# HNUicda/CoIVO

Hardware: AMD Instinct MI355X
Metric: training frame-pairs/sec at 320x256 (higher is better)
Workload: dtype bf16

## Files before the change

### coivo_amd/_lib.py

```python
from __future__ import annotations

import ctypes as C
import os

_HERE = os.path.dirname(os.path.abspath(__file__))
LIB_PATH = os.environ.get("COLVO_LIB_PATH") or os.path.join(_HERE, "lib", "libcolvo.so")

F32, BF16 = 0, 1
ABI_VERSION = 17

_vp, _i, _f, _sz = C.c_void_p, C.c_int, C.c_float, C.c_size_t


class ConvDesc(C.Structure):
    _fields_ = [(n, C.c_int32) for n in (
        "dtype", "B", "Ho", "Wo", "Cout", "ksize", "stride", "relu",
        "C0", "up0", "C1", "up1", "Hi", "Wi")]


class AdamArena(C.Structure):
    _fields_ = [("param", C.c_void_p), ("grad", C.c_void_p), ("exp_avg", C.c_void_p), ("exp_avg_sq", C.c_void_p), ("n", C.c_size_t)]


class WgradSlabs(C.Structure):
    _fields_ = [("scratch", C.c_void_p), ("dw", C.c_void_p), ("db", C.c_void_p), ("nsplit", C.c_int32), ("Cout", C.c_int32),
                ("Ctot", C.c_int32), ("pad_", C.c_int32)]


AUG_ROW_FLOATS = 20
WGRAD_GROUP_MAX = 16
MAX_ARENAS = 4
ADAM_PLAIN_PER_WG = 2048


class Cmd(C.Structure):
    _fields_ = [("op", C.c_int32), ("stream", C.c_int32), ("desc", ConvDesc), ("p", C.c_void_p * 12),
                ("i", C.c_int32 * 12), ("f", C.c_float * 4)]


(CMD_CONV_FWD, CMD_CONV_DGRAD, CMD_CONV_WGRAD, CMD_PACK_NCHW, CMD_UNPACK_NHWC_GRAD, CMD_DEPTH_HEAD_FWD,
 CMD_DEPTH_HEAD_BWD, CMD_DEPTH_HEAD_WGRAD, CMD_POSE_HEAD_FWD, CMD_POSE_HEAD_BWD, CMD_FORK, CMD_JOIN,
 CMD_DEPTH_HEAD_BWD_PARTS, CMD_CONV_DGRAD_BOTH, CMD_WGRAD_REDUCE_GROUP, CMD_CONV_DGRAD_PLANES, CMD_CONV_BWD_FUSED,
# ... 7 lines not shown
    "colvo_warp_loss_fwd": (_i, [_vp] * 7 + [_i, _i, _i, _f, _vp, _vp, _vp]),
    "colvo_warp_loss_bwd": (_i, [_vp] * 7 + [_i, _i, _i, _f] + [_vp] * 8),
    "colvo_warp_loss_fused": (_i, [_vp] * 7 + [_i, _i, _i, _f] + [_vp] * 6),
    "colvo_warp_loss_fused_bwd": (_i, [_vp] * 5 + [_i, _i, _i] + [_vp] * 5),
    "colvo_warp_loss_fused_bwd_params": (_i, [_vp] * 4 + [_i] + [_vp] * 4),
    "colvo_warp_loss_rescale": (_i, [_vp, _i, _vp]),
    "colvo_warp_loss_rescale_to": (_i, [_vp, _i, _vp, _vp]),
    "colvo_inverse_warp": (_i, [_vp] * 4 + [_i] * 4 + [_vp] * 3),
    "colvo_geo_loss_workspace_floats": (_sz, [_i, _i, _i]),
    "colvo_geo_loss_fwd": (_i, [_vp] * 4 + [_i, _i, _i] + [_vp] * 3),
    "colvo_geo_loss_bwd": (_i, [_vp] * 4 + [_i, _i, _i] + [_vp] * 7),
    "colvo_smooth_loss_fwd": (_i, [_vp, _vp, _i, _i, _i, _vp, _vp, _vp]),
    "colvo_smooth_loss_bwd": (_i, [_vp, _vp, _i, _i, _i, _vp, _vp, _vp]),
    "colvo_avgpool2_fwd": (_i, [_vp, _i, _i, _i, _vp, _vp]),
    "colvo_avgpool2_bwd": (_i, [_vp, _i, _i, _i, _vp, _vp]),
    "colvo_adam_step_multi": (_i, [_vp, _i, _f, _f, _f, _f, _f, _i, _vp]),
    "colvo_zero_multi": (_i, [_vp, _vp, _i, _vp]),
    "colvo_adam_pack_step": (_i, [_i, _vp, _i, _i, _f, _f, _f, _f, _f, _vp, _i, _vp]),
    "colvo_adam_pack_step_scaled": (_i, [_i, _vp, _i, _i, _f, _f, _f, _f, _f, _vp, _vp, _i, _vp]),
    "colvo_full_objective_workspace_floats": (_sz, [_i, _i, _i, _i]),
    "colvo_full_objective_fwd": (_i, [_vp] * 8 + [_i] * 4 + [_f] * 3 + [_vp] * 3),
    "colvo_full_objective_bwd": (_i, [_vp] * 3 + [_i] * 4 + [_f, _f] + [_vp] * 6),
    "colvo_full_objective_terms": (_i, [_vp, _i, _i, _i, _i, C.POINTER(_vp)]),
    "colvo_conv_fwd": (_i, [C.POINTER(ConvDesc)] + [_vp] * 6),
    "colvo_conv_dgrad": (_i, [C.POINTER(ConvDesc), _i, _vp, _vp, _vp, _vp, _i, _vp]),
    "colvo_conv_dgrad_both": (_i, [_vp, _vp, _vp, _vp, _vp, _vp, _vp, _vp]),
    "colvo_conv_dgrad_planes": (_i, [C.POINTER(ConvDesc), _vp, _vp, _i, _i, _vp, _i, _vp]),
    "colvo_conv_head_fused_ok": (_i, [C.POINTER(ConvDesc)]),
    "colvo_conv_head_fused": (_i, [C.POINTER(ConvDesc), _vp, _vp, _vp, _vp, _vp, _f, _f, _vp, _vp, _vp, _vp]),
    "colvo_pack_stem_pose": (_i, [_vp, _i, _i, _i, _vp, _vp, _vp]),
    "colvo_conv_bwd_fused_ok": (_i, [C.POINTER(ConvDesc)]),
    "colvo_conv_bwd_fused": (_i, [C.POINTER(ConvDesc), _vp, _vp, _vp, _i, _vp, _vp, _vp, _vp, _vp, _vp, _vp]),
    "colvo_conv_bwd_fused_head_rows": (_i, [C.POINTER(ConvDesc)]),
    "colvo_depth_head_wgrad_reduce": (_i, [_vp, _i, _vp, _vp, _vp]),
    "colvo_depth_head_wgrad_mfma_rows": (_i, [_i, _i, _i]),
    "colvo_depth_head_wgrad_mfma": (_i, [_vp, _vp, _i, _i, _i, _vp, _vp]),
    "colvo_conv_wgrad": (_i, [C.POINTER(ConvDesc)] + [_vp] * 6),
    "colvo_conv_wgrad_clean": (_i, [_vp] * 6 + [_i, _vp]),
    "colvo_conv_wgrad_scratch_bytes": (_sz, [C.POINTER(ConvDesc)]),
    "colvo_conv_wgrad_det": (_i, [C.POINTER(ConvDesc)] + [_vp] * 6 + [_sz, _vp]),
    "colvo_conv_wgrad_splits": (_i, [C.POINTER(ConvDesc)]),
    "colvo_conv_wgrad_slabs": (_i, [C.POINTER(ConvDesc)] + [_vp] * 4 + [_sz, _vp]),
    "colvo_wgrad_reduce_group": (_i, [_vp, _i, _vp]),
    "colvo_depth_head_wgrad_scratch_bytes": (_sz, [_i, _i, _i, _i]),
    "colvo_depth_head_wgrad_det": (_i, [_i, _vp, _vp, _i, _i, _i, _i, _vp, _vp, _vp, _sz, _vp]),
    "colvo_pose_head_bwd_det": (_i, [_i, _vp, _vp, _vp, _vp, _vp, _vp, _vp, _i, _i, _i, _f, _f, _vp, _vp, _vp, _vp]),
    "colvo_relu_bwd_inplace": (_i, [_i, _vp, _vp, _sz, _vp]),
    "colvo_pack_weights": (_i, [_i, _vp, _i, _i, _i, _vp, _vp, _vp]),
    "colvo_pack_weights_multi": (_i, [_i, _vp, _vp, _i, _i, _vp, _vp, _vp]),
    "colvo_pack_nchw": (_i, [_i, C.POINTER(_vp), C.POINTER(C.c_int32), _i, _i, _i, _i, _i, _vp, _vp]),
    "colvo_unpack_nhwc_grad": (_i, [_i, _vp, _i, _i, _i, _i, _i, _i, _vp, _i, _vp]),
    "colvo_depth_head_fwd": (_i, [_i, _vp, _vp, _vp, _i, _i, _i, _i, _f, _f, _vp, _vp]),
    "colvo_depth_head_bwd": (_i, [_i, _vp, _vp, _vp, _vp, _i, _i, _i, _i, _f, _f, _vp, _vp, _vp, _vp, _vp]),
    "colvo_depth_head_wgrad": (_i, [_i, _vp, _vp, _i, _i, _i, _i, _vp, _vp, _vp]),
    "colvo_depth_head_bwd_parts": (_i, [_i] + [_vp] * 9 + [_i, _i, _i, _i, _f, _f] + [_vp] * 5),
    "colvo_pose_head_fwd": (_i, [_i, _vp, _vp, _vp, _i, _i, _i, _f, _f, _vp, _vp]),
    "colvo_pose_head_bwd": (_i, [_i, _vp, _vp, _vp, _vp, _vp, _vp, _vp, _i, _i, _i, _f, _f, _vp, _vp, _vp, _vp]),
    "colvo_adam_step": (_i, [_vp, _vp, _vp, _vp, _sz, _f, _f, _f, _f, _f, _vp, _vp]),
    "colvo_adam_step_t": (_i, [_vp, _vp, _vp, _vp, _sz, _f, _f, _f, _f, _f, _i, _vp]),
    "colvo_cast_f32_bf16": (_i, [_vp, _vp, _sz, _i, _vp]),
    "colvo_zero": (_i, [_vp, _sz, _vp]),
    "colvo_frames_u8_to_f32": (_i, [_vp, _i, _i, _i, _i, _i, _vp, _vp]),
    "colvo_frames_u8_augment": (_i, [_vp, _i, _i, _i, _i, _i, _vp, _vp, _vp]),
    "colvo_read_npy_u8_frames": (_i, [_vp, _i, _i, _i, _vp, _i]),
    "colvo_backproject": (_i, [_vp, _vp, _vp, _i, _i, _i, _vp, _vp]),
    "colvo_stitch_workspace_ints": (_sz, [_i, _i, _i, _i]),
# ... 112 lines not shown
```

### coivo_amd/csrc/bwd16.hip

```cpp
#define COLVO_ACC_CONSTRAINT "+v"
#include "conv_common.h"
#include "tuning.h"

namespace colvo {
namespace {

constexpr int TOH = 8, TOW = 16, PH = TOH + 2, PW = TOW + 2, NPIX = PH * PW;
constexpr int PIXB = 32;
constexpr int WROWB = 352;

struct Bwd16K {
    const char* dy;
    const char* x;
    const char* w_bwd;
    char* dx;
    float* dw;
    float* db;
    int B, H, W;
    int tiles_x, tiles_y, ntiles, tiles_per_wg;
    int relu_mask;
    const float* dpre;
    const float* head_w;
    float* head_partials;
};

constexpr int DH = PH + 2, DW = PW + 2;

#ifndef COLVO_BWD16_HEAD_WGS
#define COLVO_BWD16_HEAD_WGS 4
#endif
template <int MODE>
__global__ __launch_bounds__(NT, MODE == 2 ? 3 : MODE == 1 ? COLVO_BWD16_HEAD_WGS : 4) void k_bwd16(const Bwd16K a) {
    constexpr bool HEAD = MODE >= 1, headw = MODE == 2;
    __shared__ __attribute__((aligned(16))) char sG[NPIX * PIXB];
    __shared__ __attribute__((aligned(16))) char sX[NPIX * PIXB];
    __shared__ __attribute__((aligned(16))) char sW[16 * WROWB];
    __shared__ float sdb[NT];
    __shared__ __attribute__((aligned(16))) uint32_t sDs[HEAD ? DH * DW : 4];
    __shared__ __attribute__((aligned(16))) float sD[MODE == 2 ? DH * DW : 4];
    __shared__ __attribute__((aligned(16))) char sY[MODE == 2 ? NPIX * PIXB : 16];
    float hb = 0.0f;
    const int tid = threadIdx.x, lane = tid & 63, wave = __builtin_amdgcn_readfirstlane(tid >> 6);
    const int l15 = lane & 15, kg = lane >> 4;

    for (int i = tid; i < 16 * 10 * 2; i += NT) {
        const int half = i & 1, tap = (i >> 1) % 10, ci = i / 20;
        u32x4 v = u32x4{0u, 0u, 0u, 0u};
        if (tap < 9) v = ld16(a.w_bwd + ((ci * 9 + tap) * 16 + half * 8) * 2);
        st16(sW + ci * WROWB + tap * 32 + half * 16, v);
    }

    const int t_begin = blockIdx.x * a.tiles_per_wg;
    const int t_end = min(a.ntiles, t_begin + a.tiles_per_wg);
    const int tiles_per_img = a.tiles_x * a.tiles_y;
    const long long img_bytes = (long long)a.H * a.W * 16 * 2;
    const long long tot_bytes = img_bytes * a.B;
    const __amdgpu_buffer_rsrc_t rdy = __builtin_amdgcn_make_buffer_rsrc((void*)a.dy, 0, (int)(tot_bytes < 0x7fffffffLL ? tot_bytes : 0x7fffffffLL), 0x00020000);
    const __amdgpu_buffer_rsrc_t rx = __builtin_amdgcn_make_buffer_rsrc((void*)a.x, 0, (int)(tot_bytes < 0x7fffffffLL ? tot_bytes : 0x7fffffffLL), 0x00020000);

    constexpr int NGRAN = 2 * NPIX * 2;
    constexpr int PPF = (NGRAN + NT - 1) / NT;
    int s_pk[PPF];
    const int s_half = tid & 1;
    auto s_which = [&](int it) -> int { const int i = it * NT + tid; return i < NPIX * 2 ? 0 : i < NGRAN ? 1 : 2; };
// ... 251 lines not shown
        }
        mfma_result_guard<bf16_t>(acc);
        {
            const int oyt = here.ty * TOH, oxt = here.tx * TOW;
#pragma unroll
            for (int mf = 0; mf < 2; ++mf) {
                const int oy = 2 * wave + mf, ox = l15;
                const int gy = oyt + oy, gx = oxt + ox;
                f32x4 v = acc[mf];
                if (a.relu_mask) {
                    const u32x2 xm = *reinterpret_cast<const u32x2*>(sX + ((oy + 1) * PW + ox + 1) * PIXB + kg * 8);
                    const uint32_t m0 = xm[0] & 0xffffu, m1 = xm[0] >> 16, m2 = xm[1] & 0xffffu, m3 = xm[1] >> 16;
                    v[0] = (m0 != 0 && m0 < 0x8000u) ? v[0] : 0.0f;
                    v[1] = (m1 != 0 && m1 < 0x8000u) ? v[1] : 0.0f;
                    v[2] = (m2 != 0 && m2 < 0x8000u) ? v[2] : 0.0f;
                    v[3] = (m3 != 0 && m3 < 0x8000u) ? v[3] : 0.0f;
                }
                if (gy < a.H && gx < a.W) {
                    u32x2 o;
                    o[0] = pack2bf(v[0], v[1]);
                    o[1] = pack2bf(v[2], v[3]);
                    *reinterpret_cast<u32x2*>(a.dx + (((long long)here.b * a.H + gy) * a.W + gx) * 32 + kg * 8) = o;
                }
            }
        }
    }

    mfma_result_guard<bf16_t>(acc);
#pragma unroll
    for (int fi = 0; fi < FPW; ++fi) {
        const int tap = wave + 4 * fi;
        if (tap < 9) {
#pragma unroll
            for (int r = 0; r < 4; ++r) atomicAdd(a.dw + ((4 * kg + r) * 9 + tap) * 16 + l15, acc[2 + fi][r]);
        }
    }
    if constexpr (headw) {
        {
            float* row = a.head_partials + ((size_t)blockIdx.x * 4 + wave) * (9 * 16 + 1);
            if (l15 < 9) {
#pragma unroll
                for (int r = 0; r < 4; ++r) row[l15 * 16 + 4 * kg + r] = acc[NACC - 1][r];
            }
            const float hbs = wave_sum(hb);
            if (lane == 0) row[9 * 16] = hbs;
        }
    }
    if (a.db) {
        __syncthreads();
        sdb[tid] = dbacc;
        __syncthreads();
        if (tid < 16) {
            float s = 0.0f;
#pragma unroll
            for (int ph = 0; ph < 16; ++ph) s += sdb[ph * 16 + tid];
            atomicAdd(a.db + tid, s);
        }
    }
}

struct HeadWgradK {
    const char* y;
    const float* dpre;
    float* partials;
    int B, H, W;
    int tiles_x, tiles_y, ntiles, tiles_per_wg;
};

__global__ __launch_bounds__(NT, 4) void k_head_wgrad_mfma(const HeadWgradK a) {
    __shared__ __attribute__((aligned(16))) char sY[TOH * TOW * PIXB];
    __shared__ __attribute__((aligned(16))) float sD[PH * PW];
    const int tid = threadIdx.x, lane = tid & 63, wave = __builtin_amdgcn_readfirstlane(tid >> 6);
    const int l15 = lane & 15, kg = lane >> 4, q = l15 >> 2, pp = lane & 3;
    const int t_begin = blockIdx.x * a.tiles_per_wg;
    const int t_end = min(a.ntiles, t_begin + a.tiles_per_wg);
    const int tiles_per_img = a.tiles_x * a.tiles_y;
    const long long img_bytes = (long long)a.H * a.W * 16 * 2;
    const long long tot_bytes = img_bytes * a.B;
    const __amdgpu_buffer_rsrc_t ry = __builtin_amdgcn_make_buffer_rsrc((void*)a.y, 0, (int)(tot_bytes < 0x7fffffffLL ? tot_bytes : 0x7fffffffLL), 0x00020000);
    const __amdgpu_buffer_rsrc_t rd = __builtin_amdgcn_make_buffer_rsrc((void*)a.dpre, 0, (int)((long long)a.B * a.H * a.W * 4), 0x00020000);
    const int g_pix = tid >> 1, g_half = tid & 1;
    const int g_oy = g_pix >> 4, g_ox = g_pix & 15;
    const int d_py = tid / PW, d_px = tid - d_py * PW;
    struct TileC { int b, ty, tx; };
    auto tile_next = [&](TileC& c) {
        if (++c.tx == a.tiles_x) { c.tx = 0; if (++c.ty == a.tiles_y) { c.ty = 0; ++c.b; } }
    };
    TileC cur;
    {
// ... 173 lines not shown
    HeadWgradK k{};
    k.y = (const char*)y; k.dpre = dpre; k.partials = partials; k.B = B; k.H = H; k.W = W;
    k.tiles_x = (W + TOW - 1) / TOW; k.tiles_y = (H + TOH - 1) / TOH; k.ntiles = B * k.tiles_x * k.tiles_y;
    const int wgs = head_wgrad_mfma_grid(B, H, W, &k.tiles_per_wg);
    colvo::launch(k_head_wgrad_mfma, dim3((unsigned)wgs), dim3(NT), 0, (hipStream_t)stream, k);
    COLVO_CHECK_LAUNCH("k_head_wgrad_mfma");
    return 0;
}

extern "C" int colvo_conv_bwd_fused_ok(const ColvoConvDesc* d) {
    if (!d) return 0;
    const long long bytes = (long long)d->B * d->Hi * d->Wi * 16 * 2;
    return d->dtype == COLVO_BF16 && d->ksize == 3 && d->stride == 1 && d->C0 == 16 && d->C1 == 0 && d->Cout == 16 && !d->up0 &&
           d->Ho == d->Hi && d->Wo == d->Wi && bytes < 0x40000000LL && TUNE(bwd16) != 0;
}

static int bwd16_grid(const ColvoConvDesc* d, int mode, int* tiles_per_wg) {
    const int ntiles = d->B * ((d->Wi + TOW - 1) / TOW) * ((d->Hi + TOH - 1) / TOH);
    int wgs = (int)TUNE(bwd16_wgs);
    const int slots = 256 * (mode == 2 ? 3 : mode == 1 ? COLVO_BWD16_HEAD_WGS : 4);
    const int want = std::min(4 * wgs, ntiles / 40);
    if (want > wgs) wgs = std::max(1, (want + slots / 2) / slots) * slots;
    if (wgs > ntiles) wgs = ntiles;
    const int tpw = (ntiles + wgs - 1) / wgs;
    if (tiles_per_wg) *tiles_per_wg = tpw;
    return (ntiles + tpw - 1) / tpw;
}

extern "C" int colvo_conv_bwd_fused_head_rows(const ColvoConvDesc* d) {
    if (!colvo_conv_bwd_fused_ok(d)) return 0;
    return 4 * bwd16_grid(d, 2, nullptr);
}

extern "C" int colvo_conv_bwd_fused(const ColvoConvDesc* d, const void* dy, const void* w_bwd, const void* x, int relu_mask, void* dx,
                                    float* dw, float* db, const float* head_dpre, const float* head_w, float* head_partials,
                                    colvo_stream_t stream) {
    COLVO_CHECK_ARG(d && dy && w_bwd && x && dx && dw && ((head_dpre == nullptr) == (head_w == nullptr)) && (!head_partials || head_dpre),
                    "colvo_conv_bwd_fused: null pointer argument");
    COLVO_CHECK_ARG(colvo_conv_bwd_fused_ok(d), "colvo_conv_bwd_fused: only bf16 16 -> 16 stride-1 layers over one directly stored source "
                                                "below 1 GiB per tensor (colvo_conv_bwd_fused_ok)");
    Bwd16K k{};
    k.dy = (const char*)dy; k.x = (const char*)x; k.w_bwd = (const char*)w_bwd; k.dx = (char*)dx; k.dw = dw; k.db = db;
    k.B = d->B; k.H = d->Hi; k.W = d->Wi; k.relu_mask = relu_mask;
    k.tiles_x = (k.W + TOW - 1) / TOW; k.tiles_y = (k.H + TOH - 1) / TOH;
    k.ntiles = k.B * k.tiles_x * k.tiles_y;
    const int wgs = bwd16_grid(d, head_partials ? 2 : head_dpre ? 1 : 0, &k.tiles_per_wg);
    k.dpre = head_dpre; k.head_w = head_w; k.head_partials = head_partials;
    form_hit(FORM_BWD16);
    if (head_partials) colvo::launch(k_bwd16<2>, dim3((unsigned)wgs), dim3(NT), 0, (hipStream_t)stream, k);
    else if (head_dpre) colvo::launch(k_bwd16<1>, dim3((unsigned)wgs), dim3(NT), 0, (hipStream_t)stream, k);
    else colvo::launch(k_bwd16<0>, dim3((unsigned)wgs), dim3(NT), 0, (hipStream_t)stream, k);
    COLVO_CHECK_LAUNCH("k_bwd16");
    return 0;
}
```

### coivo_amd/csrc/program.hip

```cpp
#include <algorithm>
#include <atomic>
#include <mutex>
#include <vector>

#include "common.h"
#include "tuning.h"

using namespace colvo;

namespace {
constexpr unsigned NEV = 256;
hipEvent_t g_ev[NEV];
std::once_flag g_ev_once;
std::atomic<unsigned> g_ev_next{0};

hipEvent_t next_event() {
    std::call_once(g_ev_once, [] {
        for (unsigned i = 0; i < NEV; ++i) (void)hipEventCreateWithFlags(&g_ev[i], hipEventDisableTiming);
    });
    return g_ev[g_ev_next.fetch_add(1, std::memory_order_relaxed) % NEV];
}

constexpr int MAX_AUX = 3;
hipStream_t g_aux[MAX_AUX] = {nullptr, nullptr, nullptr};
// ... 52 lines not shown
        case COLVO_CMD_UNPACK_NHWC_GRAD:
            return colvo_unpack_nhwc_grad(c.i[0], c.p[0], c.i[1], c.i[2], c.i[3], c.i[4], c.i[5], c.i[6], (float*)c.p[1], c.i[7], s);
        case COLVO_CMD_DEPTH_HEAD_FWD:
            return colvo_depth_head_fwd(c.i[0], c.p[0], (const float*)c.p[1], (const float*)c.p[2], c.i[1], c.i[2], c.i[3], c.i[4],
                                        c.f[0], c.f[1], (float*)c.p[3], s);
        case COLVO_CMD_DEPTH_HEAD_BWD:
            return colvo_depth_head_bwd(c.i[0], c.p[0], (const float*)c.p[1], (const float*)c.p[2], (const float*)c.p[3], c.i[1],
                                        c.i[2], c.i[3], c.i[4], c.f[0], c.f[1], (float*)c.p[4], (void*)c.p[5], (float*)c.p[6],
                                        (float*)c.p[7], s);
        case COLVO_CMD_DEPTH_HEAD_BWD_PARTS:
            return colvo_depth_head_bwd_parts(c.i[0], c.p[0], (const float*)c.p[1], (const float*)c.p[2], (const float*)c.p[3],
                                              (const float*)c.p[4], (const float*)c.p[5], (const float*)c.p[10],
                                              (const float*)c.p[6], (const float*)c.p[7],
                                              c.i[1], c.i[2], c.i[3], c.i[4], c.f[0], c.f[1], (float*)c.p[8], (void*)c.p[9], nullptr,
                                              nullptr, s);
        case COLVO_CMD_DEPTH_HEAD_WGRAD:
            if (c.p[4]) return colvo_depth_head_wgrad_det(c.i[0], c.p[0], (const float*)c.p[1], c.i[1], c.i[2], c.i[3], c.i[4],
                                                          (float*)c.p[2], (float*)c.p[3], (void*)c.p[4], (size_t)(uint32_t)c.i[5], s);
            return colvo_depth_head_wgrad(c.i[0], c.p[0], (const float*)c.p[1], c.i[1], c.i[2], c.i[3], c.i[4], (float*)c.p[2],
                                          (float*)c.p[3], s);
        case COLVO_CMD_POSE_HEAD_FWD:
            return colvo_pose_head_fwd(c.i[0], c.p[0], (const float*)c.p[1], (const float*)c.p[2], c.i[1], c.i[2], c.i[3], c.f[0],
                                       c.f[1], (float*)c.p[3], s);
        case COLVO_CMD_POSE_HEAD_BWD:
            if (c.i[4]) return colvo_pose_head_bwd_det(c.i[0], c.p[0], (const float*)c.p[1], (const float*)c.p[2], (const float*)c.p[3],
                                                       (const float*)c.p[4], (const float*)c.p[8], (const float*)c.p[9], c.i[1], c.i[2],
                                                       c.i[3], c.f[0], c.f[1], (void*)c.p[5], (float*)c.p[6], (float*)c.p[7], s);
            return colvo_pose_head_bwd(c.i[0], c.p[0], (const float*)c.p[1], (const float*)c.p[2], (const float*)c.p[3],
                                       (const float*)c.p[4], (const float*)c.p[8], (const float*)c.p[9], c.i[1], c.i[2], c.i[3],
                                       c.f[0], c.f[1], (void*)c.p[5], (float*)c.p[6], (float*)c.p[7], s);
        case COLVO_CMD_CONV_DGRAD_PLANES:
            return colvo_conv_dgrad_planes(&c.desc, c.p[0], (const float*)c.p[1], c.i[0], c.i[1], (float*)c.p[2], c.i[2], s);
        case COLVO_CMD_CONV_BWD_FUSED:
            return colvo_conv_bwd_fused(&c.desc, c.p[0], c.p[1], c.p[2], c.i[0], (void*)c.p[3], (float*)c.p[4], (float*)c.p[5],
                                        (const float*)c.p[6], (const float*)c.p[7], (float*)c.p[8], s);
        case COLVO_CMD_CONV_HEAD_FUSED:
            return colvo_conv_head_fused(&c.desc, c.p[0], c.p[1], (const float*)c.p[2], (const float*)c.p[3], (const float*)c.p[4], c.f[0],
                                         c.f[1], (void*)c.p[5], (float*)c.p[6], (void*)c.p[7], s);
        case COLVO_CMD_PACK_STEM_POSE:
            return colvo_pack_stem_pose((const float*)c.p[0], c.i[0], c.i[1], c.i[2], (void*)c.p[1], (void*)c.p[2], s);
        case COLVO_CMD_HEAD_WGRAD_MFMA:
            return colvo_depth_head_wgrad_mfma(c.p[0], (const float*)c.p[1], c.i[0], c.i[1], c.i[2], (float*)c.p[2], s);
        case COLVO_CMD_HEAD_WGRAD_REDUCE:
            return colvo_depth_head_wgrad_reduce((const float*)c.p[0], c.i[0], (float*)c.p[1], (float*)c.p[2], s);
        case COLVO_CMD_WGRAD_REDUCE_GROUP:
            return colvo_wgrad_reduce_group((const ColvoWgradSlabs*)c.p[0], c.i[0], s);
        case COLVO_CMD_SIDE_SYNC:
            return 0;
        default:
            set_error("colvo_run_commands: unknown op %d in command %d", c.op, k);
            return (int)hipErrorInvalidValue;
    }
}

extern "C" int colvo_run_command(const ColvoCmd* cmd, colvo_stream_t stream) {
    COLVO_CHECK_ARG(cmd, "colvo_run_command: null command");
    COLVO_CHECK_ARG(cmd->stream == 0, "colvo_run_command: stream selector %d (a single command runs on `stream`)", cmd->stream);
    COLVO_CHECK_ARG(cmd->op != COLVO_CMD_FORK && cmd->op != COLVO_CMD_JOIN && cmd->op != COLVO_CMD_SIDE_SYNC,
                    "colvo_run_command: op %d orders streams and needs colvo_run_commands", cmd->op);
    return run_one(*cmd, 0, stream);
}

static std::atomic<int> g_capture_policy{2};
static std::atomic<int> g_capture_group{2};
static std::atomic<int> g_capture_carry{0};

// ... 287 lines not shown
```

### coivo_amd/csrc/wgrad.hip

```cpp
#define COLVO_ACC_CONSTRAINT "+a"
#include "conv_common.h"

namespace colvo {
namespace {

template <typename T, int MT>
constexpr int dy_pitch() {
#ifdef COLVO_WGRAD_OLD_LAYOUT
    return 16 * MT * TT<T>::ES + 16;
#else
    if (TT<T>::ES == 4) return 16 * MT * 4 + 16;
    return MT == 1 ? 32 : MT == 2 ? 96 : 160;
#endif
}

template <typename T, int MT, int NG, bool TAIL, int KS = 1>
__global__ __launch_bounds__(NT * KS) void k_wgrad3x3(const WgradK a) {
    constexpr int G = TT<T>::G, ES = TT<T>::ES;
    constexpr int CK = NG * G;
    constexpr int NCOL = 9 * CK;
    constexpr int NFR = (NCOL + 15) / 16;
    constexpr int FPW = (NFR + 3) / 4;
    constexpr int PIXP = TAIL ? pitch_bytes_s2(NG * 16) : pitch_bytes(NG * 16);
    constexpr int DYP = dy_pitch<T, MT>();
// ... 385 lines not shown
    const float* slabs;
    float* dst;
    long long n4;
    int nsplit, sp;
    unsigned blk0;
};
struct ReduceGroup {
    ReduceEntry e[2 * COLVO_WGRAD_GROUP_MAX];
    int n;
};
__global__ __launch_bounds__(NT) void k_wgrad_reduce_group(const ReduceGroup g) {
    __shared__ f32x4 part[NT];
    int ei = 0;
#pragma unroll 1
    for (int i = 1; i < g.n; ++i)
        if (blockIdx.x >= g.e[i].blk0) ei = i;
    const ReduceEntry e = g.e[ei];
    const int qpb = NT / e.sp;
    const int s = threadIdx.x / qpb, ql = threadIdx.x - s * qpb;
    const long long q = (long long)(blockIdx.x - e.blk0) * qpb + ql;
    f32x4 t = f32x4{0.f, 0.f, 0.f, 0.f};
    if (q < e.n4) {
        const f32x4* base = reinterpret_cast<const f32x4*>(e.slabs) + q;
        f32x4 v[8];
        int cnt = 0;
#pragma unroll
        for (int u = 0; u < 8; ++u) {
            const int sp_i = s + u * e.sp;
            if (sp_i < e.nsplit) { v[u] = base[(long long)sp_i * e.n4]; cnt = u + 1; } else v[u] = f32x4{0.f, 0.f, 0.f, 0.f};
        }
#pragma unroll
        for (int u = 0; u < 8; ++u) t += v[u];
        (void)cnt;
        for (int sp_i = s + 8 * e.sp; sp_i < e.nsplit; sp_i += e.sp) t += base[(long long)sp_i * e.n4];
    }
    if (e.sp > 1) {
        part[threadIdx.x] = t;
        __syncthreads();
        if (s == 0) {
            for (int j = 1; j < e.sp; ++j) t += part[j * qpb + ql];
        }
    }
    if (s == 0 && q < e.n4) {
        f32x4* d = reinterpret_cast<f32x4*>(e.dst) + q;
        *d = *d + t;
    }
}

#ifdef COLVO_WTRACE
static long long* g_wtrace = nullptr;
static int g_wtrace_calls = 0;
inline WgradK wtrace_begin(WgradK k, unsigned nwg, hipStream_t s) {
    k.trace = nullptr;
    if (!getenv("COLVO_WTRACE") || nwg > (1u << 14)) return k;
    if (!g_wtrace) (void)hipMalloc(&g_wtrace, (size_t)(1u << 14) * 16 * sizeof(long long));
    (void)hipMemsetAsync(g_wtrace, 0, (size_t)nwg * 16 * sizeof(long long), s);
    k.trace = g_wtrace;
    return k;
}
inline void wtrace_end(const WgradK& k, unsigned nwg, int MT, int NG, bool tail, int ks, hipStream_t s) {
    if (!k.trace || (++g_wtrace_calls % atoi(getenv("COLVO_WTRACE"))) != 0) return;
    (void)hipStreamSynchronize(s);
    std::vector<long long> h((size_t)nwg * 16);
    (void)hipMemcpy(h.data(), g_wtrace, h.size() * sizeof(long long), hipMemcpyDeviceToHost);
    double m[16] = {0};
    long long t0 = h[0], t1 = 0;
    for (unsigned i = 0; i < nwg; ++i) {
// ... 604 lines not shown
```

### coivo_amd/nn.py

```python
from __future__ import annotations

from typing import Callable, Dict, List, Optional, Tuple

import os

import numpy as np
import torch
import torch.nn as nn

from . import _lib, ops
from .program import Program

_SIDE_PRIORITY = int(_lib.dev_env("COLVO_SIDE_PRIORITY", "-1"))

ENC_CH = (32, 64, 128, 256, 512)
DEC_CH = (16, 32, 64, 128, 256)
POSE_CH = (16, 32, 64, 128, 256, 256, 256)


class ConvParams(nn.Module):

    def __init__(self, cin: int, cout: int, k: int, cin_pad: Optional[int] = None):
        super().__init__()
        self.cin, self.cout, self.k = cin, cout, k
# ... 610 lines not shown
    def _backward_impl(self, saved, depth: torch.Tensor, d_depth: Optional[torch.Tensor], parts=None) -> None:
        A, P, inst = saved
        self._take_arena_zero()
        self.attach_grads()
        self._order_deterministic_pass()
        B, _, H, W = depth.shape
        dev = depth.device
        if parts is None:
            d_depth = d_depth.contiguous()
            ext = {"depth": depth, "d_depth": d_depth}
            which = "bwd"
        else:
            parts = tuple(_dealias([None if t is None else t.contiguous() for t in parts]))
            names = ("g_first", "g_second", "g_raw", "scale_a", "scale_b", "g_raw_second")
            ext = {"depth": depth}
            ext.update({n: t for n, t in zip(names, parts) if t is not None})
            which = "bwd:" + ",".join(n for n, t in zip(names, parts) if t is not None)

        def body():
            self._bwd_begin()

            def wgrad(name, x0, x1, dy):
                self._conv_wgrad(getattr(self, name), P[name], x0, x1, dy)

            def dgrad(name, src, dy, mask_like, dx=None, accumulate=False):
                L = getattr(self, name)
                if dx is None:
                    dx = torch.empty_like(mask_like)
                ops.conv_dgrad(P[name], src, dy, L.w_bwd, mask_like, dx, accumulate)
                return dx

            x1 = A["iconv1"]
            scratch = torch.empty(B * H * W, device=dev, dtype=torch.float32)
            fuse1 = (not self.deterministic and not self.group_wgrad and ops.conv_bwd_fused_ok(P["iconv1"]) and
                     _lib.dev_env("COLVO_NO_BWD16") is None)
            fuse_head = fuse1 and parts is not None and _lib.dev_env("COLVO_NO_BWD16_HEAD") is None
            g = None if fuse_head else torch.empty_like(x1)
            if parts is None:
                ops.depth_head_bwd(x1, self.head.w_master, depth, d_depth, scratch, g, None, None)
            else:
                ops.depth_head_bwd_parts(x1, self.head.w_master, depth, *parts[:5], scratch, g,
                                         parts[5] if len(parts) > 5 else None)
            fuse_headw = fuse_head and _lib.dev_env("COLVO_BWD16_HEADW") is not None
            if not fuse_headw:
                if (self.compute_dtype == torch.bfloat16 and ops.depth_head_wgrad_mfma_ok(B, H, W) and
                        _lib.dev_env("COLVO_NO_HEAD_WGRAD_MFMA") is None):
                    self._run_wgrad(self.head, lambda: ops.depth_head_wgrad_mfma(x1, scratch, self.head.g_master, self.head.g_bias),
                                    x1, scratch)
                else:
                    self._run_wgrad(self.head, lambda: ops.depth_head_wgrad(x1, scratch, self.head.g_master, self.head.g_bias,
                                                                            self.deterministic), x1, scratch)
            d_skip: Dict[int, torch.Tensor] = {}
            for i in range(1, 6):
                u = A[f"up{i}"]
                skip = A[f"enc{i - 1}b"] if i >= 2 else None
                Pi = P[f"iconv{i}"]
                if i == 1 and fuse1:
                    L = getattr(self, f"iconv{i}")
                    d_u = torch.empty_like(u)
                    if fuse_headw:
                        rows = ops.conv_bwd_fused_head_rows(Pi)
                        hp = torch.empty(rows * 145, device=dev, dtype=torch.float32)
                        ops.conv_bwd_fused(Pi, x1, L.w_bwd, u, True, d_u, L.g_master, L.g_bias, scratch, self.head.w_master, hp)
                        self._run_wgrad(self.head, lambda: ops.depth_head_wgrad_reduce(hp, rows, self.head.g_master, self.head.g_bias), hp)
                    elif fuse_head:
                        ops.conv_bwd_fused(Pi, x1, L.w_bwd, u, True, d_u, L.g_master, L.g_bias, scratch, self.head.w_master)
                    else:
                        ops.conv_bwd_fused(Pi, g, L.w_bwd, u, True, d_u, L.g_master, L.g_bias)
                    self._layer_done(L)
                    below = A[f"iconv{i + 1}"] if i < 5 else A["enc5b"]
                    wgrad(f"up{i}", below, None, d_u)
                    g = dgrad(f"up{i}", 0, d_u, below)
                    continue
                wgrad(f"iconv{i}", u, skip, g)
                if skip is not None:
                    L = getattr(self, f"iconv{i}")
                    d_u, d_skip[i - 1] = torch.empty_like(u), torch.empty_like(skip)
                    ops.conv_dgrad_both(P[f"iconv{i}"], g, L.w_bwd, u, skip, d_u, d_skip[i - 1])
                else:
                    d_u = dgrad(f"iconv{i}", 0, g, u)
                below = A[f"iconv{i + 1}"] if i < 5 else A["enc5b"]
                wgrad(f"up{i}", below, None, d_u)
                g = dgrad(f"up{i}", 0, d_u, below)
            for i in range(5, 0, -1):
                a = A[f"enc{i}a"]
                wgrad(f"enc{i}b", a, None, g)
                g_a = dgrad(f"enc{i}b", 0, g, a)
                src = A["in"] if i == 1 else A[f"enc{i - 1}b"]
                wgrad(f"enc{i}a", src, None, g_a)
                if i > 1:
                    g = dgrad(f"enc{i}a", 0, g_a, src, dx=d_skip[i - 1], accumulate=True)
            self._bwd_end()

        self._run_pass(inst, which, ext, body)


class _PairDepth(torch.Tensor):
    __torch_function__ = torch._C._disabled_torch_function_impl

    @staticmethod
    def wrap(full: torch.Tensor, d_t: torch.Tensor, d_r: torch.Tensor) -> "_PairDepth":
        t = full.as_subclass(_PairDepth)
# ... 230 lines not shown
```

### coivo_amd/ops.py

```python
from __future__ import annotations

import ctypes as C
from typing import Optional, Sequence, Tuple

import torch

from . import _lib, program
from ._lib import ConvDesc

MIN_DEPTH, MAX_DEPTH = 0.1, 10.0
POSE_SCALE, LCC_SCALE = 0.01, 0.1


def dt_code(dtype: torch.dtype) -> int:
    if dtype == torch.float32:
        return _lib.F32
    if dtype == torch.bfloat16:
        return _lib.BF16
    raise TypeError(f"unsupported feature-map dtype {dtype}")


def _need_cuda(*ts):
    for t in ts:
        if t is not None and not t.is_cuda:
# ... 28 lines not shown
    _need_cuda(dy, w_bwd, relu_mask, dx)
    _issue(_lib.CMD_CONV_DGRAD, d, (dy, w_bwd, relu_mask, dx), (src, int(accumulate)))


def conv_dgrad_both(d: ConvDesc, dy, w_bwd, relu_mask0, relu_mask1, dx0, dx1) -> None:
    _need_cuda(dy, w_bwd, relu_mask0, relu_mask1, dx0, dx1)
    _issue(_lib.CMD_CONV_DGRAD_BOTH, d, (dy, w_bwd, relu_mask0, relu_mask1, dx0, dx1))


def conv_dgrad_planes(d: ConvDesc, dy, w_master, c_begin: int, c_count: int, dst, accumulate: bool = False) -> None:
    _need_cuda(dy, w_master, dst)
    _issue(_lib.CMD_CONV_DGRAD_PLANES, d, (dy, w_master, dst), (c_begin, c_count, int(accumulate)))


def conv_head_fused_ok(d: ConvDesc) -> bool:
    return bool(_lib.load().colvo_conv_head_fused_ok(C.byref(d)))


def conv_head_fused(d: ConvDesc, x, w_fwd, bias, head_w, head_b, y, depth, pose_in=None) -> None:
    _need_cuda(x, w_fwd, bias, head_w, head_b, y, depth, pose_in)
    _issue(_lib.CMD_CONV_HEAD_FUSED, d, (x, w_fwd, bias, head_w, head_b, y, depth, pose_in), (), (MIN_DEPTH, MAX_DEPTH))


def pack_stem_pose(frames, stem, pose_in) -> None:
    _need_cuda(frames, stem, pose_in)
    B2, _, H, W = frames.shape
    _issue(_lib.CMD_PACK_STEM_POSE, None, (frames, stem, pose_in), (B2, H, W))


def conv_bwd_fused_ok(d: ConvDesc) -> bool:
    return bool(_lib.load().colvo_conv_bwd_fused_ok(C.byref(d)))


def conv_bwd_fused(d: ConvDesc, dy, w_bwd, x, relu_mask: bool, dx, dw, db, head_dpre=None, head_w=None, head_partials=None) -> None:
    _need_cuda(dy, w_bwd, x, dx, dw, db, head_dpre, head_w, head_partials)
    _issue(_lib.CMD_CONV_BWD_FUSED, d, (dy, w_bwd, x, dx, dw, db, head_dpre, head_w, head_partials), (int(relu_mask),))


def conv_bwd_fused_head_rows(d: ConvDesc) -> int:
    return int(_lib.load().colvo_conv_bwd_fused_head_rows(C.byref(d)))


def depth_head_wgrad_mfma_ok(B: int, H: int, W: int) -> bool:
    return _lib.load().colvo_depth_head_wgrad_mfma_rows(B, H, W) > 0


def depth_head_wgrad_mfma(y, dpre, dw, db) -> None:
    _need_cuda(y, dpre, dw, db)
    B, H, W, Cc = y.shape
    if Cc != 16 or y.dtype != torch.bfloat16:
        raise ValueError("depth_head_wgrad_mfma: the 16-channel bf16 head only")
    lib = _lib.load()
    rows = lib.colvo_depth_head_wgrad_mfma_rows(B, H, W)
    if rows <= 0:
        raise RuntimeError("colvo_depth_head_wgrad_mfma_rows failed")
    hp = torch.empty(rows * 145, device=y.device, dtype=torch.float32)
    _issue(_lib.CMD_HEAD_WGRAD_MFMA, None, (y, dpre, hp), (B, H, W))
    _issue(_lib.CMD_HEAD_WGRAD_REDUCE, None, (hp, dw, db), (int(rows),))


def depth_head_wgrad_reduce(partials, rows: int, dw, db) -> None:
    _need_cuda(partials, dw, db)
    _issue(_lib.CMD_HEAD_WGRAD_REDUCE, None, (partials, dw, db), (int(rows),))


def conv_wgrad_scratch(d: ConvDesc, device) -> torch.Tensor:
    n = _lib.load().colvo_conv_wgrad_scratch_bytes(C.byref(d))
    if n == 0:
        raise RuntimeError("colvo_conv_wgrad_scratch_bytes failed: " + _lib.load().colvo_last_error().decode("utf-8", "replace"))
# ... 182 lines not shown
```

### include/colvo.h

```cpp
#ifndef COLVO_H_
#define COLVO_H_

#include <stddef.h>
#include <stdint.h>

#ifdef __cplusplus
extern "C" {
#endif

#define COLVO_ABI_VERSION 17

typedef void* colvo_stream_t;

enum { COLVO_F32 = 0, COLVO_BF16 = 1 };

int colvo_abi_version(void);
const char* colvo_last_error(void);


size_t colvo_warp_loss_workspace_floats(int B, int H, int W);

int colvo_warp_loss_fwd(const float* tgt, const float* ref, const float* depth, const float* pose,
                        const float* K, const float* lcc_a, const float* lcc_b,
                        int B, int H, int W, float ssim_weight,
                        float* workspace, float* loss_state, colvo_stream_t stream);

int colvo_warp_loss_bwd(const float* tgt, const float* ref, const float* depth, const float* pose,
                        const float* K, const float* lcc_a, const float* lcc_b,
                        int B, int H, int W, float ssim_weight,
                        const float* loss_state, const float* grad_loss,
                        float* workspace, float* d_depth, float* d_pose, float* d_a, float* d_b,
                        colvo_stream_t stream);

int colvo_warp_loss_fused(const float* tgt, const float* ref, const float* depth, const float* pose,
                          const float* K, const float* lcc_a, const float* lcc_b,
                          int B, int H, int W, float ssim_weight,
                          float* workspace, float* loss_state, float* d_depth_raw, float* grad_partials,
                          float* grad_unit, colvo_stream_t stream);
int colvo_warp_loss_fused_bwd(const float* loss_state, const float* grad_loss, const float* d_depth_raw,
                              const float* grad_partials, const float* pose, int B, int H, int W,
                              float* d_depth, float* d_pose, float* d_a, float* d_b, colvo_stream_t stream);
int colvo_warp_loss_fused_bwd_params(const float* loss_state, const float* grad_loss, const float* grad_partials,
                                     const float* pose, int B, float* d_pose, float* d_a, float* d_b,
// ... 35 lines not shown
    int32_t Ho, Wo;
    int32_t Cout;
    int32_t ksize;
    int32_t stride;
    int32_t relu;
    int32_t C0;
    int32_t up0;
    int32_t C1;
    int32_t up1;
    int32_t Hi, Wi;
} ColvoConvDesc;

int colvo_conv_fwd(const ColvoConvDesc* d, const void* x0, const void* x1, const void* w_fwd,
                   const float* bias, void* y, colvo_stream_t stream);

int colvo_conv_dgrad(const ColvoConvDesc* d, int src, const void* dy, const void* w_bwd,
                     const void* relu_mask, void* dx, int accumulate, colvo_stream_t stream);
int colvo_conv_dgrad_both(const ColvoConvDesc* d, const void* dy, const void* w_bwd, const void* relu_mask0,
                          const void* relu_mask1, void* dx0, void* dx1, colvo_stream_t stream);

int colvo_conv_dgrad_planes(const ColvoConvDesc* d, const void* dy, const float* w_master, int c_begin, int c_count, float* dst,
                            int accumulate, colvo_stream_t stream);

int colvo_conv_head_fused_ok(const ColvoConvDesc* d);
int colvo_conv_head_fused(const ColvoConvDesc* d, const void* x, const void* w_fwd, const float* bias, const float* head_w,
                          const float* head_b, float min_depth, float max_depth, void* y, float* depth, void* pose_in,
                          colvo_stream_t stream);
int colvo_pack_stem_pose(const float* frames, int B2, int H, int W, void* stem, void* pose_in, colvo_stream_t stream);

int colvo_conv_bwd_fused_ok(const ColvoConvDesc* d);
int colvo_conv_bwd_fused(const ColvoConvDesc* d, const void* dy, const void* w_bwd, const void* x, int relu_mask, void* dx, float* dw,
                         float* db, const float* head_dpre, const float* head_w, float* head_partials, colvo_stream_t stream);
int colvo_conv_bwd_fused_head_rows(const ColvoConvDesc* d);
int colvo_depth_head_wgrad_reduce(const float* partials, int rows, float* dw, float* db, colvo_stream_t stream);
int colvo_depth_head_wgrad_mfma_rows(int B, int H, int W);
int colvo_depth_head_wgrad_mfma(const void* y, const float* dpre, int B, int H, int W, float* partials, colvo_stream_t stream);

int colvo_conv_wgrad(const ColvoConvDesc* d, const void* x0, const void* x1, const void* dy,
                     float* dw, float* db, colvo_stream_t stream);
int colvo_conv_wgrad_clean(const ColvoConvDesc* d, const void* x0, const void* x1, const void* dy,
                           float* dw, float* db, int arena_is_zero, colvo_stream_t stream);

size_t colvo_conv_wgrad_scratch_bytes(const ColvoConvDesc* d);
int colvo_conv_wgrad_det(const ColvoConvDesc* d, const void* x0, const void* x1, const void* dy, float* dw, float* db,
                         void* scratch, size_t scratch_bytes, colvo_stream_t stream);
#define COLVO_WGRAD_GROUP_MAX 16
typedef struct ColvoWgradSlabs {
    const void* scratch;
    float* dw;
    float* db;
    int32_t nsplit, Cout, Ctot, pad_;
} ColvoWgradSlabs;
int colvo_conv_wgrad_splits(const ColvoConvDesc* d);
int colvo_conv_wgrad_slabs(const ColvoConvDesc* d, const void* x0, const void* x1, const void* dy, void* scratch,
                           size_t scratch_bytes, colvo_stream_t stream);
int colvo_wgrad_reduce_group(const ColvoWgradSlabs* sets, int n, colvo_stream_t stream);
size_t colvo_depth_head_wgrad_scratch_bytes(int B, int H, int W, int C);
int colvo_depth_head_wgrad_det(int dtype, const void* x, const float* dpre, int B, int H, int W, int C, float* dw, float* db,
                               void* scratch, size_t scratch_bytes, colvo_stream_t stream);
int colvo_pose_head_bwd_det(int dtype, const void* x, const float* w, const float* d_pose, const float* d_a, const float* d_b,
                            const float* scale_a, const float* scale_b, int B, int HW, int C, float pose_scale, float lcc_scale,
                            void* dx, float* dw, float* db, colvo_stream_t stream);

int colvo_relu_bwd_inplace(int dtype, const void* y, void* dy, size_t n, colvo_stream_t stream);

int colvo_pack_weights(int dtype, const float* w_master, int Cout, int kk, int Cin,
// ... 187 lines not shown
```

Before: 5574.

## Enable fused 16-channel conv backward in deterministic mode via per-block slab reduction

Adds a slab variant of the fused 16->16 conv backward kernel. Each workgroup writes its weight and bias gradient partials to its own scratch slab instead of using float atomics, and a separate group reduction then sums the slabs in a fixed order. The iconv1 fused path, previously turned off in deterministic mode, can now run there, and the wgrad reduction can overlap through the side-stream wgrad runner. The slab-reduce loop is also unrolled to issue eight loads at a time. The cost is extra scratch memory and an additional reduce launch, and whether it runs depends on the deterministic setting.

```diff
diff --git a/coivo_amd/_lib.py b/coivo_amd/_lib.py
--- a/coivo_amd/_lib.py
+++ b/coivo_amd/_lib.py
@@ -7,7 +7,7 @@
 LIB_PATH = os.environ.get("COLVO_LIB_PATH") or os.path.join(_HERE, "lib", "libcolvo.so")
 
 F32, BF16 = 0, 1
-ABI_VERSION = 17
+ABI_VERSION = 18
 
 _vp, _i, _f, _sz = C.c_void_p, C.c_int, C.c_float, C.c_size_t
 
@@ -81,6 +81,8 @@
     "colvo_conv_bwd_fused_ok": (_i, [C.POINTER(ConvDesc)]),
     "colvo_conv_bwd_fused": (_i, [C.POINTER(ConvDesc), _vp, _vp, _vp, _i, _vp, _vp, _vp, _vp, _vp, _vp, _vp]),
     "colvo_conv_bwd_fused_head_rows": (_i, [C.POINTER(ConvDesc)]),
+    "colvo_conv_bwd_fused_scratch_bytes": (_sz, [C.POINTER(ConvDesc), _i]),
+    "colvo_conv_bwd_fused_det": (_i, [C.POINTER(ConvDesc), _vp, _vp, _vp, _i, _vp, _vp, _vp, _vp, _vp, _vp, _vp, _sz, _vp]),
     "colvo_depth_head_wgrad_reduce": (_i, [_vp, _i, _vp, _vp, _vp]),
     "colvo_depth_head_wgrad_mfma_rows": (_i, [_i, _i, _i]),
     "colvo_depth_head_wgrad_mfma": (_i, [_vp, _vp, _i, _i, _i, _vp, _vp]),
diff --git a/coivo_amd/csrc/bwd16.hip b/coivo_amd/csrc/bwd16.hip
--- a/coivo_amd/csrc/bwd16.hip
+++ b/coivo_amd/csrc/bwd16.hip
@@ -22,6 +22,7 @@
     const float* dpre;
     const float* head_w;
     float* head_partials;
+    float* slabs;
 };
 
 constexpr int DH = PH + 2, DW = PW + 2;
@@ -29,7 +30,7 @@
 #ifndef COLVO_BWD16_HEAD_WGS
 #define COLVO_BWD16_HEAD_WGS 4
 #endif
-template <int MODE>
+template <int MODE, bool SLAB = false>
 __global__ __launch_bounds__(NT, MODE == 2 ? 3 : MODE == 1 ? COLVO_BWD16_HEAD_WGS : 4) void k_bwd16(const Bwd16K a) {
     constexpr bool HEAD = MODE >= 1, headw = MODE == 2;
     __shared__ __attribute__((aligned(16))) char sG[NPIX * PIXB];
@@ -347,7 +348,11 @@
         const int tap = wave + 4 * fi;
         if (tap < 9) {
 #pragma unroll
-            for (int r = 0; r < 4; ++r) atomicAdd(a.dw + ((4 * kg + r) * 9 + tap) * 16 + l15, acc[2 + fi][r]);
+            for (int r = 0; r < 4; ++r) {
+                const int e = ((4 * kg + r) * 9 + tap) * 16 + l15;
+                if constexpr (SLAB) a.slabs[(size_t)blockIdx.x * (16 * 9 * 16) + e] = acc[2 + fi][r];
+                else atomicAdd(a.dw + e, acc[2 + fi][r]);
+            }
         }
     }
     if constexpr (headw) {
@@ -361,7 +366,7 @@
             if (lane == 0) row[9 * 16] = hbs;
         }
     }
-    if (a.db) {
+    if (SLAB || a.db) {
         __syncthreads();
         sdb[tid] = dbacc;
         __syncthreads();
@@ -369,7 +374,8 @@
             float s = 0.0f;
 #pragma unroll
             for (int ph = 0; ph < 16; ++ph) s += sdb[ph * 16 + tid];
-            atomicAdd(a.db + tid, s);
+            if constexpr (SLAB) a.slabs[(size_t)gridDim.x * (16 * 9 * 16) + (size_t)blockIdx.x * 16 + tid] = s;
+            else atomicAdd(a.db + tid, s);
         }
     }
 }
@@ -609,6 +615,27 @@
     return 4 * bwd16_grid(d, 2, nullptr);
 }
 
+static int bwd16_launch(const ColvoConvDesc* d, const void* dy, const void* w_bwd, const void* x, int relu_mask, void* dx, float* dw,
+                        float* db, const float* head_dpre, const float* head_w, float* head_partials, float* slabs, int* rows,
+                        hipStream_t stream) {
+    Bwd16K k{};
+    k.dy = (const char*)dy; k.x = (const char*)x; k.w_bwd = (const char*)w_bwd; k.dx = (char*)dx; k.dw = dw; k.db = db;
+    k.B = d->B; k.H = d->Hi; k.W = d->Wi; k.relu_mask = relu_mask;
+    k.tiles_x = (k.W + TOW - 1) / TOW; k.tiles_y = (k.H + TOH - 1) / TOH;
+    k.ntiles = k.B * k.tiles_x * k.tiles_y;
+    const int wgs = bwd16_grid(d, head_partials ? 2 : head_dpre ? 1 : 0, &k.tiles_per_wg);
+    k.dpre = head_dpre; k.head_w = head_w; k.head_partials = head_partials; k.slabs = slabs;
+    if (rows) *rows = wgs;
+    form_hit(FORM_BWD16);
+    if (slabs && head_dpre) colvo::launch(k_bwd16<1, true>, dim3((unsigned)wgs), dim3(NT), 0, stream, k);
+    else if (slabs) colvo::launch(k_bwd16<0, true>, dim3((unsigned)wgs), dim3(NT), 0, stream, k);
+    else if (head_partials) colvo::launch(k_bwd16<2>, dim3((unsigned)wgs), dim3(NT), 0, stream, k);
+    else if (head_dpre) colvo::launch(k_bwd16<1>, dim3((unsigned)wgs), dim3(NT), 0, stream, k);
+    else colvo::launch(k_bwd16<0>, dim3((unsigned)wgs), dim3(NT), 0, stream, k);
+    COLVO_CHECK_LAUNCH("k_bwd16");
+    return 0;
+}
+
 extern "C" int colvo_conv_bwd_fused(const ColvoConvDesc* d, const void* dy, const void* w_bwd, const void* x, int relu_mask, void* dx,
                                     float* dw, float* db, const float* head_dpre, const float* head_w, float* head_partials,
                                     colvo_stream_t stream) {
@@ -616,17 +643,32 @@
                     "colvo_conv_bwd_fused: null pointer argument");
     COLVO_CHECK_ARG(colvo_conv_bwd_fused_ok(d), "colvo_conv_bwd_fused: only bf16 16 -> 16 stride-1 layers over one directly stored source "
                                                 "below 1 GiB per tensor (colvo_conv_bwd_fused_ok)");
-    Bwd16K k{};
-    k.dy = (const char*)dy; k.x = (const char*)x; k.w_bwd = (const char*)w_bwd; k.dx = (char*)dx; k.dw = dw; k.db = db;
-    k.B = d->B; k.H = d->Hi; k.W = d->Wi; k.relu_mask = relu_mask;
-    k.tiles_x = (k.W + TOW - 1) / TOW; k.tiles_y = (k.H + TOH - 1) / TOH;
-    k.ntiles = k.B * k.tiles_x * k.tiles_y;
-    const int wgs = bwd16_grid(d, head_partials ? 2 : head_dpre ? 1 : 0, &k.tiles_per_wg);
-    k.dpre = head_dpre; k.head_w = head_w; k.head_partials = head_partials;
-    form_hit(FORM_BWD16);
-    if (head_partials) colvo::launch(k_bwd16<2>, dim3((unsigned)wgs), dim3(NT), 0, (hipStream_t)stream, k);
-    else if (head_dpre) colvo::launch(k_bwd16<1>, dim3((unsigned)wgs), dim3(NT), 0, (hipStream_t)stream, k);
-    else colvo::launch(k_bwd16<0>, dim3((unsigned)wgs), dim3(NT), 0, (hipStream_t)stream, k);
-    COLVO_CHECK_LAUNCH("k_bwd16");
-    return 0;
-}
+    return bwd16_launch(d, dy, w_bwd, x, relu_mask, dx, dw, db, head_dpre, head_w, head_partials, nullptr, nullptr, (hipStream_t)stream);
+}
+
+extern "C" size_t colvo_conv_bwd_fused_scratch_bytes(const ColvoConvDesc* d, int mode) {
+    if (!colvo_conv_bwd_fused_ok(d) || mode < 0 || mode > 1) return 0;
+    return (size_t)bwd16_grid(d, mode, nullptr) * (16 * 9 * 16 + 16) * sizeof(float);
+}
+
+extern "C" int colvo_conv_bwd_fused_det(const ColvoConvDesc* d, const void* dy, const void* w_bwd, const void* x, int relu_mask, void* dx,
+                                        float* dw, float* db, const float* head_dpre, const float* head_w, float* head_partials,
+                                        void* scratch, size_t scratch_bytes, colvo_stream_t stream) {
+    COLVO_CHECK_ARG(d && dy && w_bwd && x && dx && scratch && ((head_dpre == nullptr) == (head_w == nullptr)),
+                    "colvo_conv_bwd_fused_det: null pointer argument");
+    COLVO_CHECK_ARG(!head_partials, "colvo_conv_bwd_fused_det: the head's own weight gradient (head_partials) has no slab form");
+    COLVO_CHECK_ARG(colvo_conv_bwd_fused_ok(d), "colvo_conv_bwd_fused_det: only bf16 16 -> 16 stride-1 layers over one directly stored "
+                                                "source below 1 GiB per tensor (colvo_conv_bwd_fused_ok)");
+    const size_t need = colvo_conv_bwd_fused_scratch_bytes(d, head_dpre ? 1 : 0);
+    COLVO_CHECK_ARG(scratch_bytes >= need, "colvo_conv_bwd_fused_det: scratch of %zu bytes, %zu needed (colvo_conv_bwd_fused_scratch_bytes)",
+                    scratch_bytes, need);
+    COLVO_CHECK_ARG(((uintptr_t)scratch % 16) == 0 && ((uintptr_t)dw % 16) == 0 && ((uintptr_t)db % 16) == 0,
+                    "colvo_conv_bwd_fused_det: scratch, dw and db must be 16-byte aligned");
+    int rows = 0;
+    if (int e = bwd16_launch(d, dy, w_bwd, x, relu_mask, dx, dw, db, head_dpre, head_w, nullptr, (float*)scratch, &rows, (hipStream_t)stream))
+        return e;
+    if (!dw) return 0;
+    ColvoWgradSlabs set{};
+    set.scratch = scratch; set.dw = dw; set.db = db; set.nsplit = rows; set.Cout = 16; set.Ctot = 16;
+    return colvo_wgrad_reduce_group(&set, 1, stream);
+}
diff --git a/coivo_amd/csrc/program.hip b/coivo_amd/csrc/program.hip
--- a/coivo_amd/csrc/program.hip
+++ b/coivo_amd/csrc/program.hip
@@ -108,6 +108,9 @@
         case COLVO_CMD_CONV_DGRAD_PLANES:
             return colvo_conv_dgrad_planes(&c.desc, c.p[0], (const float*)c.p[1], c.i[0], c.i[1], (float*)c.p[2], c.i[2], s);
         case COLVO_CMD_CONV_BWD_FUSED:
+            if (c.p[9]) return colvo_conv_bwd_fused_det(&c.desc, c.p[0], c.p[1], c.p[2], c.i[0], (void*)c.p[3], (float*)c.p[4], (float*)c.p[5],
+                                                        (const float*)c.p[6], (const float*)c.p[7], (float*)c.p[8], (void*)c.p[9],
+                                                        (size_t)(uint32_t)c.i[1], s);
             return colvo_conv_bwd_fused(&c.desc, c.p[0], c.p[1], c.p[2], c.i[0], (void*)c.p[3], (float*)c.p[4], (float*)c.p[5],
                                         (const float*)c.p[6], (const float*)c.p[7], (float*)c.p[8], s);
         case COLVO_CMD_CONV_HEAD_FUSED:
diff --git a/coivo_amd/csrc/wgrad.hip b/coivo_amd/csrc/wgrad.hip
--- a/coivo_amd/csrc/wgrad.hip
+++ b/coivo_amd/csrc/wgrad.hip
@@ -441,7 +441,16 @@
 #pragma unroll
         for (int u = 0; u < 8; ++u) t += v[u];
         (void)cnt;
-        for (int sp_i = s + 8 * e.sp; sp_i < e.nsplit; sp_i += e.sp) t += base[(long long)sp_i * e.n4];
+        for (int sp0 = s + 8 * e.sp; sp0 < e.nsplit; sp0 += 8 * e.sp) {
+#pragma unroll
+            for (int u = 0; u < 8; ++u) {
+                const int sp_i = sp0 + u * e.sp;
+                if (sp_i < e.nsplit) v[u] = base[(long long)sp_i * e.n4];
+            }
+#pragma unroll
+            for (int u = 0; u < 8; ++u)
+                if (sp0 + u * e.sp < e.nsplit) t += v[u];
+        }
     }
     if (e.sp > 1) {
         part[threadIdx.x] = t;
diff --git a/coivo_amd/nn.py b/coivo_amd/nn.py
--- a/coivo_amd/nn.py
+++ b/coivo_amd/nn.py
@@ -666,16 +666,16 @@
 
             x1 = A["iconv1"]
             scratch = torch.empty(B * H * W, device=dev, dtype=torch.float32)
-            fuse1 = (not self.deterministic and not self.group_wgrad and ops.conv_bwd_fused_ok(P["iconv1"]) and
-                     _lib.dev_env("COLVO_NO_BWD16") is None)
-            fuse_head = fuse1 and parts is not None and _lib.dev_env("COLVO_NO_BWD16_HEAD") is None
+            fuse1 = (not self.group_wgrad and ops.conv_bwd_fused_ok(P["iconv1"]) and _lib.dev_env("COLVO_NO_BWD16") is None)
+            fuse_head = (fuse1 and parts is not None and _lib.dev_env("COLVO_NO_BWD16_HEAD") is None and
+                         (not self.deterministic or _lib.dev_env("COLVO_DET_BWD16_HEAD") is not None))
             g = None if fuse_head else torch.empty_like(x1)
             if parts is None:
                 ops.depth_head_bwd(x1, self.head.w_master, depth, d_depth, scratch, g, None, None)
             else:
                 ops.depth_head_bwd_parts(x1, self.head.w_master, depth, *parts[:5], scratch, g,
                                          parts[5] if len(parts) > 5 else None)
-            fuse_headw = fuse_head and _lib.dev_env("COLVO_BWD16_HEADW") is not None
+            fuse_headw = fuse_head and not self.deterministic and _lib.dev_env("COLVO_BWD16_HEADW") is not None
             if not fuse_headw:
                 if (self.compute_dtype == torch.bfloat16 and ops.depth_head_wgrad_mfma_ok(B, H, W) and
                         _lib.dev_env("COLVO_NO_HEAD_WGRAD_MFMA") is None):
@@ -692,16 +692,25 @@
                 if i == 1 and fuse1:
                     L = getattr(self, f"iconv{i}")
                     d_u = torch.empty_like(u)
+                    side_sum = False
                     if fuse_headw:
                         rows = ops.conv_bwd_fused_head_rows(Pi)
                         hp = torch.empty(rows * 145, device=dev, dtype=torch.float32)
                         ops.conv_bwd_fused(Pi, x1, L.w_bwd, u, True, d_u, L.g_master, L.g_bias, scratch, self.head.w_master, hp)
                         self._run_wgrad(self.head, lambda: ops.depth_head_wgrad_reduce(hp, rows, self.head.g_master, self.head.g_bias), hp)
-                    elif fuse_head:
-                        ops.conv_bwd_fused(Pi, x1, L.w_bwd, u, True, d_u, L.g_master, L.g_bias, scratch, self.head.w_master)
                     else:
-                        ops.conv_bwd_fused(Pi, g, L.w_bwd, u, True, d_u, L.g_master, L.g_bias)
-                    self._layer_done(L)
+                        rows = ops.conv_bwd_fused_scratch(Pi, 1 if fuse_head else 0, dev) if self.deterministic else None
+                        side_sum = rows is not None and _lib.dev_env("COLVO_DET_BWD16_MAIN") is None
+                        dw1 = None if side_sum else L.g_master
+                        if fuse_head:
+                            ops.conv_bwd_fused(Pi, x1, L.w_bwd, u, True, d_u, dw1, L.g_bias, scratch, self.head.w_master, scratch=rows)
+                        else:
+                            ops.conv_bwd_fused(Pi, g, L.w_bwd, u, True, d_u, dw1, L.g_bias, scratch=rows)
+                    if side_sum:
+                        sets = [(rows, L.g_master, L.g_bias, rows.numel() // (16 * 9 * 16 + 16), 16, 16)]
+                        self._run_wgrad(L, lambda: ops.wgrad_reduce_group(sets), rows)
+                    else:
+                        self._layer_done(L)
                     below = A[f"iconv{i + 1}"] if i < 5 else A["enc5b"]
                     wgrad(f"up{i}", below, None, d_u)
                     g = dgrad(f"up{i}", 0, d_u, below)
diff --git a/coivo_amd/ops.py b/coivo_amd/ops.py
--- a/coivo_amd/ops.py
+++ b/coivo_amd/ops.py
@@ -84,9 +84,18 @@
     return bool(_lib.load().colvo_conv_bwd_fused_ok(C.byref(d)))
 
 
-def conv_bwd_fused(d: ConvDesc, dy, w_bwd, x, relu_mask: bool, dx, dw, db, head_dpre=None, head_w=None, head_partials=None) -> None:
-    _need_cuda(dy, w_bwd, x, dx, dw, db, head_dpre, head_w, head_partials)
-    _issue(_lib.CMD_CONV_BWD_FUSED, d, (dy, w_bwd, x, dx, dw, db, head_dpre, head_w, head_partials), (int(relu_mask),))
+def conv_bwd_fused(d: ConvDesc, dy, w_bwd, x, relu_mask: bool, dx, dw, db, head_dpre=None, head_w=None, head_partials=None,
+                   scratch: Optional[torch.Tensor] = None) -> None:
+    _need_cuda(dy, w_bwd, x, dx, dw, db, head_dpre, head_w, head_partials, scratch)
+    nb = 0 if scratch is None else scratch.numel() * scratch.element_size()
+    _issue(_lib.CMD_CONV_BWD_FUSED, d, (dy, w_bwd, x, dx, dw, db, head_dpre, head_w, head_partials, scratch), (int(relu_mask), nb))
+
+
+def conv_bwd_fused_scratch(d: ConvDesc, mode: int, device) -> torch.Tensor:
+    n = _lib.load().colvo_conv_bwd_fused_scratch_bytes(C.byref(d), int(mode))
+    if n == 0:
+        raise RuntimeError("colvo_conv_bwd_fused_scratch_bytes: the layer or the mode has no deterministic fused backward")
+    return torch.empty(n // 4, device=device, dtype=torch.float32)
 
 
 def conv_bwd_fused_head_rows(d: ConvDesc) -> int:
diff --git a/include/colvo.h b/include/colvo.h
--- a/include/colvo.h
+++ b/include/colvo.h
@@ -8,7 +8,7 @@
 extern "C" {
 #endif
 
-#define COLVO_ABI_VERSION 17
+#define COLVO_ABI_VERSION 18
 
 typedef void* colvo_stream_t;
 
@@ -110,6 +110,10 @@
 int colvo_conv_bwd_fused(const ColvoConvDesc* d, const void* dy, const void* w_bwd, const void* x, int relu_mask, void* dx, float* dw,
                          float* db, const float* head_dpre, const float* head_w, float* head_partials, colvo_stream_t stream);
 int colvo_conv_bwd_fused_head_rows(const ColvoConvDesc* d);
+size_t colvo_conv_bwd_fused_scratch_bytes(const ColvoConvDesc* d, int mode);
+int colvo_conv_bwd_fused_det(const ColvoConvDesc* d, const void* dy, const void* w_bwd, const void* x, int relu_mask, void* dx,
+                             float* dw, float* db, const float* head_dpre, const float* head_w, float* head_partials, void* scratch,
+                             size_t scratch_bytes, colvo_stream_t stream);
 int colvo_depth_head_wgrad_reduce(const float* partials, int rows, float* dw, float* db, colvo_stream_t stream);
 int colvo_depth_head_wgrad_mfma_rows(int B, int H, int W);
 int colvo_depth_head_wgrad_mfma(const void* y, const float* dpre, int B, int H, int W, float* partials, colvo_stream_t stream);
```

Result: faster. 5691, median of 6 (+2.1%).
